# audexdev/Lossless-Audio-Codec

Measured on AMD Instinct MI355X. Metric: encode Msamples/s at 1/2/4/8 MI355X; byte-identical .lac vs CPU ref, higher is better.
Workload: dtype int64

## Files before the change

lossless-audio-codec_amd/csrc/analyze_core.h:

```cpp
#pragma once
#include <type_traits>

#include "lacx_types.h"
#include "x87.h"

namespace lacx {

template <int CH_, int T_>
struct Geo {
    static constexpr int CH = CH_;
    static constexpr int T = T_;
    static constexpr int MAXN = CH_ * T_;
    static constexpr int LV = (CH_ == 16) ? 5 : ((CH_ == 8) ? 4 : 3);
    static constexpr int TPG = 64 / CH_;
    static constexpr int NG = MAXN / 64;
    static constexpr int W256 = 256 / CH_;
    static constexpr int W96 = 96 / CH_;
    static constexpr int MAXP = (MAXN >= 8192) ? 8 : ((MAXN >= 4096) ? 7 : ((MAXN >= 2048) ? 6 : ((MAXN >= 1024) ? 5 : ((MAXN >= 512) ? 4 : 3))));
    static constexpr int NSEG = (2 << MAXP) - 2;
    static constexpr int SW = (T_ < 64) ? T_ : 64;
    static constexpr int NW = (T_ + 63) / 64;
    static_assert(32 % CH_ == 0, "chunk must divide the 96/256 windows");
    static_assert(MAXN % 64 == 0, "whole groups");
};
// ... 788 lines not shown
        if (ZR) {
            n1 = n2;
            n2 = n3;
            n3 = peek_u<G>(sh, (uint32_t)(a + i) + 4u, n);
        }
    }
    ChunkCosts out;
    out.rice = rice;
    out.bin = bin;
    out.zr = zr;
    out.hasrun = hasrun;
    return out;
}

template <class G, bool NARROW, bool ZR = true, bool FULL = false, bool STEADY = false>
LACX_HD void phase_b(Thread<G>& th, const Smem<G>& sh, uint32_t k0) {
    const ChunkCosts cc = phase_b_span<G, NARROW, ZR, FULL ? G::CH : 0, STEADY>(sh, th.n, th.tid, 0, th.cnt, k0);
    th.crice = cc.rice;
    th.cbin = cc.bin;
    th.czr = cc.zr;
    th.chasrun = cc.hasrun;
}

template <class G>
LACX_HD void phase_b_dispatch(Thread<G>& th, const Smem<G>& sh, uint32_t k0, bool narrow, bool zr, bool full, bool steady) {
    auto go = [&](auto narrow_t, auto zr_t) {
        constexpr bool N = decltype(narrow_t)::value, Z = decltype(zr_t)::value;
        if (full) {
            if (steady) phase_b<G, N, Z, true, true>(th, sh, k0); else phase_b<G, N, Z, true, false>(th, sh, k0);
        } else {
            if (steady) phase_b<G, N, Z, false, true>(th, sh, k0); else phase_b<G, N, Z, false, false>(th, sh, k0);
        }
    };
    if (narrow) {
        if (zr) go(std::true_type{}, std::true_type{}); else go(std::true_type{}, std::false_type{});
    } else {
        if (zr) go(std::false_type{}, std::true_type{}); else go(std::false_type{}, std::false_type{});
    }
}
template <class G>
LACX_HD void phase_b_dispatch(Thread<G>& th, const Smem<G>& sh, uint32_t k0, bool narrow, bool zr, bool full) {
    phase_b_dispatch<G>(th, sh, k0, narrow, zr, full, G::T > 64 && th.tid >= 64 && 64 * G::CH >= 256);
}

#ifndef LACX_QUEUED_STEADY
#define LACX_QUEUED_STEADY 1
#endif
template <class G>
LACX_HD void phase_b_queued(Thread<G>& th, const Smem<G>& sh, int t, uint32_t k0, bool narrow, bool zr, bool full) {
    Thread<G> c;
    thread_init(c, th.n, t);
    phase_b_dispatch<G>(c, sh, k0, narrow, zr, full, LACX_QUEUED_STEADY != 0);
    th.crice += c.crice;
    th.cbin += c.cbin;
    th.czr += c.czr;
    th.chasrun |= c.chasrun;
}

LACX_HD uint32_t census_code(uint32_t u);
LACX_HD uint32_t census_shift_sum(uint32_t cen, uint32_t K);

struct RunShape {
    uint32_t nin4, tokens, hasrun, first_in4;
};
template <int CH>
LACX_HD RunShape run_shape(uint32_t E, int32_t f) {
    RunShape r{0u, 0u, 0u, 0u};
#pragma unroll
    for (int i = 0; i < CH; ++i) {
        const uint32_t z = (E >> i) & 1u;
        f = (f + 1) & (int32_t)(0u - z);
        const uint32_t after = E >> (i + 1);
        const uint32_t ahead = (after & 1u) == 0u ? 0u : ((after & 2u) == 0u ? 1u : ((after & 4u) == 0u ? 2u : 3u));
        const uint32_t in4 = z & flag01((uint32_t)f + ahead >= 4u);
        const uint32_t runend = in4 & ((after & 1u) ^ 1u);
        r.nin4 += in4;
        r.tokens += (5u + (((uint32_t)(f - 4)) >> 2)) & (0u - runend);
        r.hasrun |= runend;
        if (i == 0) r.first_in4 = in4;
    }
    return r;
}

template <class G, bool NARROW, bool ZR>
LACX_HD bool phase_b_quick(Thread<G>& th, const Smem<G>& sh) {
    if constexpr (G::T <= 64 || 64 * G::CH <= 256) {
        return false;
    } else {
        const int t = th.tid;
        if (t < 64 || th.cnt != G::CH) return false;
        using Sum = typename std::conditional<NARROW, uint32_t, uint64_t>::type;
        const Sum P0 = (Sum)sh.tabP[t], P1 = (Sum)sh.tabP[t + 1];
        const Sum W0 = (Sum)sh.tabP[t - G::W256], W1 = (Sum)sh.tabP[t - G::W256 + 1];
        const uint32_t c0 = (uint32_t)th.a, c1 = c0 + (uint32_t)G::CH;
        const uint32_t km = kmean_t<NARROW>(P0, c1);
        uint32_t ok = flag01(km == kmean_t<NARROW>(P1, c0));
        const uint32_t Llo = (uint32_t)(((P0 - W1) + 128u) >> 8), Lhi = (uint32_t)(((P1 - W0) + 128u) >> 8);
        const uint32_t Ulo = (3u * Llo + 3u) >> 2, Uhi = (3u * Lhi + 3u) >> 2;
        const uint32_t Dlo = Llo + (Llo + 3u) / 3u + 1u, Dhi = Lhi + (Lhi + 3u) / 3u + 1u;
        const uint64_t Xlo = NARROW ? (uint64_t)((uint32_t)P0 + (c0 >> 1)) : (uint64_t)P0 + (c0 >> 1);
        const uint64_t Xhi = NARROW ? (uint64_t)((uint32_t)P1 + (c1 >> 1)) : (uint64_t)P1 + (c1 >> 1);
        const uint32_t act_never = flag01(Xhi < (uint64_t)c0), act_always = flag01(Xlo >= (uint64_t)c1);
        const uint32_t up_always = flag01(Xhi < (uint64_t)Ulo * c0), up_never = flag01(Xlo >= (uint64_t)Uhi * c1);
        const uint32_t dn_always = flag01(Xlo >= (uint64_t)Dhi * c1), dn_never = flag01(Xhi < (uint64_t)Dlo * c0);
        ok &= act_never | (act_always & (up_always | up_never) & (dn_always | dn_never));
        const int32_t drift = (int32_t)((act_never ^ 1u) & up_always) - (int32_t)((act_never ^ 1u) & dn_always);
        const uint32_t d0 = window_flags<G>(sh.tabF, t), din = sh.tabF[t], dout = sh.tabF[t - G::W96];
        const int32_t l0 = (int32_t)(d0 & 0xFFFFu), z0 = (int32_t)(d0 >> 16);
        const uint32_t big_always = flag01(l0 - (int32_t)(dout & 0xFFFFu) >= 72), big_never = flag01(l0 + (int32_t)(din & 0xFFFFu) < 72);
        uint32_t sml_always, sml_never;
        {
            const uint32_t zin = sh.tabZM[t], zout = sh.tabZM[t - G::W96];
            int32_t z = z0, zmin = z0, zmax = z0;
#pragma unroll
            for (int i = 0; i + 1 < G::CH; ++i) {
                z += (int32_t)((zin >> i) & 1u) - (int32_t)((zout >> i) & 1u);
                zmin = z < zmin ? z : zmin;
                zmax = z > zmax ? z : zmax;
            }
            sml_always = flag01(zmin >= 77);
            sml_never = flag01(zmax < 77);
        }
        ok &= big_always | (big_never & (sml_always | sml_never));
        int32_t bias = drift + (int32_t)big_always - (int32_t)((big_always ^ 1u) & sml_always);
        bias = bias < -1 ? -1 : (bias > 1 ? 1 : bias);
        int bk = (int)km + bias;
        bk = bk < 0 ? 0 : (bk > 31 ? 31 : bk);
        const uint32_t k = (uint32_t)bk;
        uint32_t any = 0;
        Sum ksum = 0;
#pragma unroll
        for (int l = 0; l < G::LV; ++l) {
            any |= th.cs[l];
            ksum += (Sum)(th.cs[l] >> k) << l;
        }
        if (ZR) ok &= flag01((any >> ((k + 3u) < 24u ? (k + 3u) : 24u)) == 0u);
        if (ok == 0u) return false;
        const Sum rice = ksum + (uint32_t)G::CH * (1u + k);
        uint32_t n14 = 0, nbig = (uint32_t)G::CH, small_shifted = 0;
        if (th.umin <= 4u) {
            uint32_t cen = 0;
#pragma unroll
            for (int i = 0; i < G::CH; ++i) cen += census_code(sh.u[i * G::T + t] & 0x3FFFFFFFu);
            n14 = ((cen >> 5) & 31u) + ((cen >> 10) & 31u) + ((cen >> 15) & 31u) + ((cen >> 20) & 31u);
            nbig = (cen >> 25) & 31u;
            small_shifted = census_shift_sum(cen, k);
        }
        th.crice = rice;
        th.cbin = (Sum)(2u * (uint32_t)G::CH + n14 + nbig * (1u + k)) + (ksum - small_shifted);
        RunShape rs{0u, 0u, 0u, 0u};
        if (ZR && th.zmask != 0u)
            rs = run_shape<G::CH>(th.zmask | (((uint32_t)sh.tabUZ[t + 1] & 7u) << G::CH), th.a - 1 - sh.tabNZ[t]);
        const uint32_t nin4 = rs.nin4, tokens = rs.tokens, hasrun = rs.hasrun;
        th.czr = ksum + (Sum)(((uint32_t)G::CH - nin4) * (3u + k) + tokens);
        th.chasrun = hasrun;
        return true;
    }
}

template <class G>
LACX_HD bool phase_b_quick_dispatch(Thread<G>& th, const Smem<G>& sh, bool narrow, bool zr) {
    if (narrow) return zr ? phase_b_quick<G, true, true>(th, sh) : phase_b_quick<G, true, false>(th, sh);
    return zr ? phase_b_quick<G, false, true>(th, sh) : phase_b_quick<G, false, false>(th, sh);
}

LACX_HD uint64_t candidate_lower_bound(uint32_t g_sum, uint32_t aux_sum, uint32_t ends, uint32_t n, int zero_run) {
// ... 611 lines not shown
```

lossless-audio-codec_amd/csrc/device_util.h:

```cpp
#pragma once
#include <hip/hip_runtime.h>

#include "analyze_core.h"
#include "kernels.h"

namespace lacx {

#ifdef LACX_STAMPS
extern __device__ unsigned long long g_stamp_acc[40];
#define STAMP(k)                                                        \
    do {                                                                \
        const unsigned long long _now = __builtin_amdgcn_s_memtime();   \
        stamp_acc[k] += _now - stamp_prev;                              \
        stamp_prev = _now;                                              \
    } while (0)
#define STAMP_PARAMS , unsigned long long* stamp_acc, unsigned long long& stamp_prev
#define STAMP_ARGS , stamp_acc, stamp_prev
#else
#define STAMP(k) do { } while (0)
#define STAMP_PARAMS
#define STAMP_ARGS
#endif
constexpr int kDppRowShr1 = 0x111, kDppRowShr2 = 0x112, kDppRowShr4 = 0x114, kDppRowShr8 = 0x118;
constexpr int kDppRowBcast15 = 0x142, kDppRowBcast31 = 0x143;
// ... 111 lines not shown
    v |= dpp_mov<kDppRowShr2, 0xF>(0u, v);
    v |= dpp_mov<kDppRowShr4, 0xF>(0u, v);
    v |= dpp_mov<kDppRowShr8, 0xF>(0u, v);
    v |= dpp_mov<kDppRowBcast15, 0xA>(0u, v);
    return v;
}
__device__ __forceinline__ uint64_t half_scan_min_u64(uint64_t v) {
    auto step = [](uint64_t a, uint32_t lo, uint32_t hi) {
        const uint64_t b = ((uint64_t)hi << 32) | lo;
        return b < a ? b : a;
    };
#define LACX_MIN_STEP(CTRL, MASK) \
    v = step(v, dpp_mov<CTRL, MASK>(0xFFFFFFFFu, (uint32_t)v), dpp_mov<CTRL, MASK>(0xFFFFFFFFu, (uint32_t)(v >> 32)))
    LACX_MIN_STEP(kDppRowShr1, 0xF);
    LACX_MIN_STEP(kDppRowShr2, 0xF);
    LACX_MIN_STEP(kDppRowShr4, 0xF);
    LACX_MIN_STEP(kDppRowShr8, 0xF);
    LACX_MIN_STEP(kDppRowBcast15, 0xA);
#undef LACX_MIN_STEP
    return v;
}
__device__ __forceinline__ uint64_t half_sum_u64(uint64_t v) { return half_last_u64(half_scan_add_u64(v)); }
__device__ __forceinline__ uint32_t half_sum_u32(uint32_t v) { return half_last_u32(half_scan_add_u32(v)); }
__device__ __forceinline__ uint32_t half_or_u32(uint32_t v) { return half_last_u32(half_scan_or_u32(v)); }
template <int SW> constexpr auto slot_last_u32 = SW == 64 ? &wave_last_u32 : &half_last_u32;
template <int SW> constexpr auto slot_last_u64 = SW == 64 ? &wave_last_u64 : &half_last_u64;
template <int SW> constexpr auto slot_scan_add_u32 = SW == 64 ? &wave_scan_add_u32 : &half_scan_add_u32;
template <int SW> constexpr auto slot_scan_add_u64 = SW == 64 ? &wave_scan_add_u64 : &half_scan_add_u64;
template <int SW> constexpr auto slot_scan_max_i32 = SW == 64 ? &wave_scan_max_i32 : &half_scan_max_i32;
template <int SW> constexpr auto slot_scan_or_u32 = SW == 64 ? &wave_scan_or_u32 : &half_scan_or_u32;
template <int SW> constexpr auto slot_scan_min_u64 = SW == 64 ? &wave_scan_min_u64 : &half_scan_min_u64;
template <int SW> constexpr auto slot_sum_u64 = SW == 64 ? &wave_sum_u64 : &half_sum_u64;
template <int SW> constexpr auto slot_sum_u32 = SW == 64 ? &wave_sum_u32 : &half_sum_u32;
template <int SW> constexpr auto slot_or_u32 = SW == 64 ? &wave_or_u32 : &half_or_u32;
template <int SW>
__device__ __forceinline__ uint32_t slot_first_u32(uint32_t v) {
    static_assert(SW == 64 || SW == 32, "the wave or one of its halves");
    if constexpr (SW == 64) {
        return (uint32_t)__builtin_amdgcn_readfirstlane((int)v);
    } else {
        const uint32_t lo = (uint32_t)__builtin_amdgcn_readlane((int)v, 0), hi = (uint32_t)__builtin_amdgcn_readlane((int)v, 32);
        return upper_half() ? hi : lo;
    }
}
template <int SW>
__device__ __forceinline__ uint64_t slot_ballot(bool pred) {
    const unsigned long long m = __ballot(pred);
    if constexpr (SW == 64) {
        return m;
    } else {
        return upper_half() ? (uint32_t)(m >> 32) : (uint32_t)m;
    }
}
template <int SW>
__device__ __forceinline__ uint32_t slot_rank(uint64_t m) {
    if constexpr (SW == 64) {
        return __builtin_amdgcn_mbcnt_hi((uint32_t)(m >> 32), __builtin_amdgcn_mbcnt_lo((uint32_t)m, 0u));
    } else {
        return (uint32_t)__popc((uint32_t)m & ((1u << (threadIdx.x & 31u)) - 1u));
    }
}

template <int LOG>
__device__ __forceinline__ uint32_t seg_sum_u32(uint32_t v) {
    if (LOG >= 1) v += dpp_mov<kDppRowShr1, 0xF>(0u, v);
    if (LOG >= 2) v += dpp_mov<kDppRowShr2, 0xF>(0u, v);
    if (LOG >= 3) v += dpp_mov<kDppRowShr4, 0xF>(0u, v);
    if (LOG >= 4) v += dpp_mov<kDppRowShr8, 0xF>(0u, v);
    if (LOG >= 5) v += dpp_mov<kDppRowBcast15, 0xA>(0u, v);
    if (LOG >= 6) v += dpp_mov<kDppRowBcast31, 0xC>(0u, v);
    return v;
}
__device__ __forceinline__ uint32_t seg_sum_u32(uint32_t v, int log2_lanes) {
    switch (log2_lanes) {
        case 1: return seg_sum_u32<1>(v);
        case 2: return seg_sum_u32<2>(v);
        case 3: return seg_sum_u32<3>(v);
        case 4: return seg_sum_u32<4>(v);
        case 5: return seg_sum_u32<5>(v);
        default: return seg_sum_u32<6>(v);
    }
}

template <class G>
struct ScanRegs {
    uint64_t v, inc;
    int32_t z, zinc;
};

template <class G, class M>
__device__ __forceinline__ void scan_pz_part1(M& sh, int tid, ScanRegs<G>& r) {
    const int lane = tid & 63, wave = tid >> 6;
    r.v = sh.tabP[tid];
    r.z = sh.tabNZ[tid];
    const uint64_t inc = slot_scan_add_u64<G::SW>(r.v);
    const int32_t zinc = slot_scan_max_i32<G::SW>(r.z);
    r.inc = inc;
    r.zinc = zinc;
    if (lane == G::SW - 1) {
        sh.wtotP[wave] = inc;
        sh.wtotZ[wave] = zinc;
    }
}

template <class G, class M>
__device__ __forceinline__ uint64_t scan_pz_part2(M& sh, int tid, const ScanRegs<G>& r) {
    const int lane = tid & 63, wave = tid >> 6;
    uint64_t base = 0, total = 0;
    int32_t zbase = -1;
#pragma unroll
    for (int w = 0; w < G::NW; ++w) {
        const uint64_t pw = sh.wtotP[w];
        const int32_t z = sh.wtotZ[w];
        total += pw;
        if (w < wave) {
            base += pw;
            zbase = z > zbase ? z : zbase;
        }
    }
    int32_t zprev = __shfl_up(r.zinc, 1, G::SW);
    if (lane == 0) zprev = -1;
    sh.tabP[tid] = base + r.inc - r.v;
    sh.tabNZ[tid] = zprev > zbase ? zprev : zbase;
    if (tid == G::T - 1) {
        sh.tabP[G::T] = base + r.inc;
        sh.tabNZ[G::T] = r.zinc > zbase ? r.zinc : zbase;
    }
    return total;
}

template <class G>
__device__ __forceinline__ void plane_totals_wave(const Thread<G>& th, uint32_t* planeTot, uint32_t* planeTot256,
                                                  int tid, int first_plane = 0) {
    const int lane = tid & 63, wave = tid >> 6;
    uint32_t any = 0;
#pragma unroll
    for (int l = 0; l < G::LV; ++l) any |= th.cs[l];
    if constexpr (G::SW == 32) {
        const int nplanes = 32 - __clz((int)slot_or_u32<32>(any));
        uint32_t mine = 0;
        for (int b = 0; b < nplanes; ++b) {
            uint32_t tot = 0;
#pragma unroll
            for (int l = 0; l < G::LV; ++l) tot += (uint32_t)__popc((uint32_t)slot_ballot<32>((th.cs[l] >> b) & 1u)) << l;
            if (lane == b) mine = tot;
        }
        static_assert(G::SW != 32 || G::W256 == G::SW, "the slot is its own first 256 samples");
        if (lane < nplanes) {
            if (lane >= first_plane) atomicAdd(&planeTot[lane], mine);
            atomicAdd(&planeTot256[lane], mine);
        }
        return;
    }
    const int nplanes = 32 - __clz((int)wave_or_u32(any));
    const uint64_t m256 = (G::W256 >= 64) ? ~0ull : ((1ull << (G::W256 & 63)) - 1ull);
    uint32_t mine = 0, mine256 = 0;
    const bool first256 = wave == 0;
    for (int b = first256 ? 0 : first_plane; b < nplanes; ++b) {
        uint32_t tot = 0, tot256 = 0;
#pragma unroll
        for (int l = 0; l < G::LV; ++l) {
            const uint64_t m = __ballot((th.cs[l] >> b) & 1u);
            tot += (uint32_t)__popcll(m) << l;
            if (first256) tot256 += (uint32_t)__popcll(m & m256) << l;
        }
        if (lane == b) {
// ... 176 lines not shown
```

lossless-audio-codec_amd/csrc/k_analyze.hip:

```cpp
#include <hip/hip_runtime.h>

#include <cstdlib>
#include <mutex>

#include "emit_device.h"
#include "kernels_internal.h"

namespace lacx {

#ifdef LACX_STAMPS
__device__ unsigned long long g_stamp_acc[40];
#endif

#ifdef LACX_TEST_HOOKS
#define LACX_HOOK(prm, bits) (((prm).debug_skip & (bits)) != 0u)
#else
#define LACX_HOOK(prm, bits) false
#endif

struct PendingSlot {
    long long idx;
    uint32_t done, silent;
};

// ... 46 lines not shown
            }
            asm volatile("s_waitcnt vmcnt(0)" ::: "memory");
            __syncthreads();
            if (tid == 0) __hip_atomic_store(&t->state, tmpl_key, __ATOMIC_RELEASE, __HIP_MEMORY_SCOPE_AGENT);
        }
    }
    if (defer) {
        if (tid == 0) {
            defer->idx = idx;
            defer->done = done ? 1u : 0u;
            defer->silent = LACX_HOOK(prm, 8192u) ? 1u : 0u;
        }
        return;
    }
    asm volatile("s_waitcnt vmcnt(0)" ::: "memory");
    __syncthreads();
    if (tid == 0) {
        if (done) fa.emitted[idx] = 2u;
        if (!LACX_HOOK(prm, 8192u)) rec_store(&fa.ready_rec[idx], done ? 1ull : 2ull);
    }
}

__device__ __forceinline__ void publish_pending(const FuseArgs& fa, PendingSlot& pend, int tid) {
    if (tid == 0) {
        const long long idx = pend.idx;
        if (idx >= 0) {
            if (pend.done) fa.emitted[idx] = 2u;
            if (!pend.silent) rec_store(&fa.ready_rec[idx], pend.done ? 1ull : 2ull);
        }
        pend.idx = -1;
    }
}

template <class G>
__device__ __forceinline__ void score_candidate_wave(Smem<G>& sh, int cand, uint32_t n, int zero_run, uint32_t k0,
                                                     const uint32_t* planeTot, const unsigned long long* acc, int lane,
                                                     bool ksums, uint32_t kmask) {
    uint64_t key = ~0ull;
    if (ksums) {
        if (lane < 16 && ((kmask >> lane) & 1u)) key = (((uint64_t)planeTot[lane] + (uint64_t)n * (uint64_t)(1 + lane)) << 4) | (uint64_t)lane;
    } else {
        const int b = 29 - lane;
        const uint64_t w = (lane < 30) ? ((uint64_t)planeTot[b] << b) : 0ull;
        const uint64_t tk = slot_scan_add_u64<G::SW>(w);
        if (lane >= 14 && lane < 30 && ((kmask >> b) & 1u)) key = (((tk >> b) + (uint64_t)n * (uint64_t)(1 + b)) << 4) | (uint64_t)b;
    }
    const uint64_t best_key = slot_last_u64<G::SW>(slot_scan_min_u64<G::SW>(key));
    if (lane == 0) {
        const uint64_t sbits = best_key >> 4;
        const uint32_t sk = (uint32_t)(best_key & 15u);
        const uint64_t rice = acc[0], bin = acc[1];
        const uint32_t hasrun = acc[3] != 0;
        const uint64_t zr = (zero_run && hasrun) ? acc[2] : rice;
        const uint64_t a = rice < sbits ? rice : sbits;
        const uint64_t c = zr < bin ? zr : bin;
        const uint64_t best = a < c ? a : c;
        if (sh.best_cand < 0 || best < sh.best_bits || (best == sh.best_bits && cand < sh.best_cand)) {
            sh.best_cand = cand;
            sh.best_bits = best;
            sh.best_rice = rice;
            sh.best_zr = zr;
            sh.best_bin = bin;
            sh.best_static = sbits;
            sh.best_k0 = k0;
            sh.best_sk = sk;
            sh.best_hasrun = hasrun;
        }
    }
}

template <int SW>
__device__ __forceinline__ uint32_t initial_k_wave(const uint32_t* planes256, uint32_t n, int lane, bool ksums) {
    const uint32_t m = n < 256u ? n : 256u;
    uint64_t key = ~0ull;
    if (ksums) {
        if (lane <= 12) key = (((uint64_t)planes256[lane] + (uint64_t)m * (uint64_t)(1 + lane)) << 4) | (uint64_t)lane;
    } else {
        const int b = 29 - lane;
        const uint64_t w = (lane < 30) ? ((uint64_t)planes256[b] << b) : 0ull;
        const uint64_t tk = slot_scan_add_u64<SW>(w);
        if (lane >= 17 && lane < 30) key = (((tk >> b) + (uint64_t)m * (uint64_t)(1 + b)) << 4) | (uint64_t)b;
    }
    return (uint32_t)(slot_last_u64<SW>(slot_scan_min_u64<SW>(key)) & 15u);
}

template <class G>
__device__ __forceinline__ void slot_sync() {
    if constexpr (G::T <= 64) {
        asm volatile("s_waitcnt lgkmcnt(0)" ::: "memory");
    } else {
        __syncthreads();
    }
}

template <class G>
__device__ __forceinline__ void analyze_slot(unsigned char* smem_raw, const AnalyzeParams& prm, uint32_t n_in,
                                             const SlotSrc& src, int64_t start, const LpcSet* __restrict__ lpc_slot,
                                             ChannelPlan* __restrict__ plan_out, int tid, const FuseArgs& fuse,
                                             const long long fuse_idx, const bool fuse_flag_byte,
                                             const uint32_t fuse_flag_value, PendingSlot* pend) {
    Smem<G>& sh = *reinterpret_cast<Smem<G>*>(smem_raw);
    const uint32_t n = n_in;
#ifdef LACX_STAMPS
    unsigned long long stamp_acc[40];
    for (int k = 0; k < 40; ++k) stamp_acc[k] = 0;
    unsigned long long stamp_prev = __builtin_amdgcn_s_memtime();
    const unsigned long long stamp_rt0 = __builtin_amdgcn_s_memrealtime();
#endif
    Thread<G> th;
    thread_init(th, n, tid);
    const uint32_t chunk_bits = stage_samples(th, sh, src, start);
    {
        const bool wave_silent = slot_ballot<G::SW>(chunk_bits != 0u) == 0ull;
        if ((tid & 63) == 0) sh.wtotF[tid >> 6] = wave_silent ? 0u : 1u;
    }
    for (int i = tid; i < (int)(sizeof(LpcSet) / 2); i += G::T)
        reinterpret_cast<uint16_t*>(&sh.lpc)[i] = reinterpret_cast<const uint16_t*>(lpc_slot)[i];
    if (tid < 32) {
        sh.planeTot[0][tid] = sh.planeTot[1][tid] = 0;
        sh.planeTot256[0][tid] = sh.planeTot256[1][tid] = 0;
    }
    if (tid < 4) sh.acc[0][tid] = sh.acc[1][tid] = 0;
    if constexpr (G::T >= 33) {
        if (tid < 33) (&sh.lbacc[0][0])[tid] = 0;
    } else {
        for (int i = tid; i < 33; i += G::T) (&sh.lbacc[0][0])[i] = 0;
    }
    if (tid < 2) sh.has4[tid] = 0;
    if (tid == 0) {
        sh.best_cand = -1;
        sh.tabUZ[G::T] = sh.tabUZ[G::T + 1] = 0;
    }
    if (pend) asm volatile("s_waitcnt vmcnt(0)" ::: "memory");
    slot_sync<G>();
    if (pend) publish_pending(fuse, *pend, tid);
    STAMP(0);

    auto run_pass1 = [&](const bool real) {
        asm volatile("" : "+v"(th.a));
        const bool lpc_off = LACX_HOOK(prm, 16u);
        const uint32_t per_thread = 34u * (uint32_t)G::CH;
        const int32_t left = (int32_t)n - (int32_t)((tid >> 6) * 64 * G::CH);
        const uint32_t valid = left <= 0 ? 0u : (left >= G::SW * G::CH ? (uint32_t)(G::SW * G::CH) : (uint32_t)left);
        const uint32_t beyond = (uint32_t)(G::SW * G::CH) - valid;
        auto reduce_pair = [&](int c0, const BoundPartials& b0, bool two, const BoundPartials& b1) {
            const uint32_t lo = per_thread - b0.msum, hi = two ? per_thread - b1.msum : 0u;
            const uint32_t g2 = slot_sum_u32<G::SW>(lo | (hi << 16));
            const uint32_t cnt0 = slot_sum_u32<G::SW>(bound_counts<G::CH>(b0));
            const uint32_t cnt1 = two ? slot_sum_u32<G::SW>(bound_counts<G::CH>(b1)) : 0u;
            if ((tid & 63) == 0 && real) {
#pragma unroll
                for (int h = 0; h < 2; ++h) {
                    if (h == 0 || two) {
                        const uint32_t g = h ? (g2 >> 16) : (g2 & 0xFFFFu);
                        const uint32_t cnt = h ? cnt1 : cnt0;
                        const uint32_t nz = cnt & 0x7FFu, n4 = (cnt >> 11) & 0x7FFu, ends = cnt >> 22;
                        atomicAdd(&sh.lbacc[c0 + h][0], g - nz - beyond);
                        atomicAdd(&sh.lbacc[c0 + h][1], (nz - beyond) + (n4 << 16));
                        atomicAdd(&sh.lbacc[c0 + h][2], ends);
                    }
                }
            }
        };
        {
            BoundPartials bf[6];
            if (n == (uint32_t)G::MAXN) pass1_bounds_fixed<G, true>(th, sh, bf);
// ... 117 lines not shown
                sh.bqcount = 0;
                int next = best_key == ~0ull ? -1 : (int)(best_key & 15u);
                if (next >= 0 && !LACX_HOOK(prm, 128u) && candidate_pruned(best_key >> 4, next, sh.best_bits, sh.best_cand)) next = -1;
                sh.next_cand = next;
            }
        }
        STAMP(1);
        slot_sync<G>();
        STAMP(4);
        const int cand = sh.next_cand;
        if (cand < 0) break;
        tried |= 1u << cand;
        asm volatile("" : "+v"(th.a));
        uint32_t* pt = sh.planeTot[parity];
        uint32_t* pt256 = sh.planeTot256[parity];
        unsigned long long* acc = sh.acc[parity];
        {
            uint32_t ures[G::CH];
            phase_r_residual(th, sh, cand, ures);
            phase_r_store(th, sh, ures);
        }
        ScanRegs<G> sr;
        scan_pz_part1(sh, tid, sr);
        STAMP(3);
        slot_sync<G>();
        const uint64_t total_u = scan_pz_part2(sh, tid, sr);
        const bool narrow = total_u < kNarrowLimit;
        const bool ksums = narrow && !LACX_HOOK(prm, 262144u);
        const uint32_t kmask = !LACX_HOOK(prm, 1048576u) ? static_k_candidates<G::SW>(total_u, n, tid & 63) : 0xFFFFu;
        if (!LACX_HOOK(prm, 1u)) {
            if (ksums) ksums_wave(th, pt, pt256, tid, kmask);
            else plane_totals_wave(th, pt, pt256, tid, kmask ? (int)__builtin_ctz(kmask) : 0);
        }
        if (tid < 64) {
            const uint32_t k0w = initial_k_wave<G::SW>(pt256, n, tid, ksums);
            if (tid == 0) sh.cur_k0 = k0w;
        }
        STAMP(6);
        if (LACX_HOOK(prm, 2u)) {
            sh.tabF[tid] = 0;
            th.has4 = 1u;
        } else if (narrow) {
            phase_a<G, true>(th, sh);
        } else {
            phase_a<G, false>(th, sh);
        }
        if (slot_ballot<G::SW>(th.has4 != 0u) != 0ull && (tid & 63) == 0) sh.has4[parity] = 1u;
        STAMP(8);
        slot_sync<G>();
        STAMP(10);
        const uint32_t k0 = sh.cur_k0;
        asm volatile("" : "+v"(th.tid));
        if (LACX_HOOK(prm, 4u)) {
            th.crice = th.cbin = th.czr = 1;
            th.chasrun = 0;
        } else {
            const bool zr = prm.zero_run && sh.has4[parity] != 0u;
            const bool full = n == (uint32_t)G::MAXN;
            if (G::T <= 64 || LACX_HOOK(prm, 524288u)) {
                phase_b_dispatch<G>(th, sh, k0, narrow, zr, full);
                if ((uint32_t)th.a >= n) {
                    th.crice = th.cbin = th.czr = 0;
                    th.chasrun = 0;
                }
            } else {
                const bool live = (uint32_t)th.a < n;
                bool quick = false;
                if (tid >= 64 && live) quick = phase_b_quick_dispatch<G>(th, sh, narrow, zr);
                if (!quick) {
                    th.crice = th.cbin = th.czr = 0;
                    th.chasrun = 0;
                }
                if (tid >= 64) {
                    const unsigned long long slow = __ballot(live && !quick);
                    if (slow != 0ull) {
                        uint32_t base = 0;
                        if ((tid & 63) == 0) base = atomicAdd(&sh.bqcount, (uint32_t)__popcll(slow));
                        base = (uint32_t)__builtin_amdgcn_readfirstlane((int)base);
                        if (live && !quick) sh.bqueue[base + __builtin_amdgcn_mbcnt_hi((uint32_t)(slow >> 32), __builtin_amdgcn_mbcnt_lo((uint32_t)slow, 0u))] = (uint16_t)tid;
                    }
                }
                STAMP(11);
                slot_sync<G>();
                if (tid < 64) {
                    if (live) phase_b_dispatch<G>(th, sh, k0, narrow, zr, full, false);
                } else {
                    const int w = tid >> 6;
                    const int order = (w & 3) ? (w - 1 - (w >> 2)) : (11 + (w >> 2));
                    const uint32_t qn = sh.bqcount;
                    for (uint32_t e0 = (uint32_t)order * 64u; e0 < qn; e0 += 15u * 64u) {
                        const uint32_t e = e0 + (uint32_t)(tid & 63);
                        if (e < qn) phase_b_queued<G>(th, sh, (int)sh.bqueue[e], k0, narrow, zr, full);
                    }
                }
            }
        }
        STAMP(12);
        {
            const uint64_t r0 = slot_sum_u64<G::SW>(th.crice);
            const uint64_t r1 = slot_sum_u64<G::SW>(th.cbin);
            const uint64_t r2 = slot_sum_u64<G::SW>(th.czr);
            const uint32_t r3 = slot_or_u32<G::SW>(th.chasrun);
            if ((tid & 63) == 0) {
                atomicAdd(&acc[0], (unsigned long long)r0);
                atomicAdd(&acc[1], (unsigned long long)r1);
                atomicAdd(&acc[2], (unsigned long long)r2);
                atomicAdd(&acc[3], (unsigned long long)r3);
            }
        }
        STAMP(13);
        slot_sync<G>();
        STAMP(14);
        pending = cand;
        pending_k0 = k0;
        pending_ksums = ksums;
        pending_kmask = kmask;
        parity ^= 1;
    }

    STAMP(15);
    asm volatile("" : "+v"(tid), "+v"(th.tid), "+v"(th.a));
    const int best = sh.best_cand;
    int max_p = 0;
    if (prm.partitioning && n >= (uint32_t)kMinPartition) max_p = max_partition_order(n);
    const int nseg = max_p > 0 ? ((2 << max_p) - 2) : 0;
    PartMem<G>& pm = sh.xp.part;
    auto clear_partition_scratch = [&]() {
        for (int i = tid; i < nseg; i += G::T) {
            pm.segacc[i][0] = pm.segacc[i][1] = pm.segacc[i][2] = 0;
            pm.segrun[i] = 0;
        }
        if (tid <= G::MAXP) pm.pbits[tid] = 0;
    };
    if (best == pending && !LACX_HOOK(prm, 16384u)) {
        clear_partition_scratch();
        slot_sync<G>();
    } else {
        phase_r(th, sh, best);
        ScanRegs<G> sr;
        scan_pz_part1(sh, tid, sr);
        slot_sync<G>();
        clear_partition_scratch();
        scan_pz_part2(sh, tid, sr);
        slot_sync<G>();
    }
    const bool pnarrow = sh.tabP[G::T] < kNarrowLimit;
    STAMP(16);
    if (max_p > 0) {
        {
            constexpr int kLog = G::TPG == 4 ? 2 : (G::TPG == 8 ? 3 : 4);
            static_assert(G::TPG == 4 || G::TPG == 8 || G::TPG == 16, "lanes per 64-sample group");
            uint32_t words[15];
            packed_planes(th, words);
            const bool last = (tid & (G::TPG - 1)) == G::TPG - 1;
#pragma unroll
            for (int w = 0; w < 15; ++w) {
                const uint32_t v = seg_sum_u32<kLog>(words[w]);
                if (last) pm.grp[w][tid / G::TPG] = v;
            }
            if (tid < 15) pm.grp[tid][G::NG] = 0;
        }
        slot_sync<G>();
        {
            constexpr int NW = G::NW;
            const int wave = tid >> 6, lane = tid & 63;
            for (int w = wave; w < 15; w += NW) wave_exclusive_scan_u32<G::SW>(pm.grp[w], G::NG + 1, lane);
        }
// ... 475 lines not shown
```

Baseline: 24950.

## Split phase-B slow-path chunks across four-lane quads for CH16 narrow slots

For 16-sample chunks in the narrow path, the queued slow-path chunk cost evaluation (plus the first 64 chunks) is redistributed so that each chunk is handled by a quad of four lanes, each lane taking four samples. Prefix sums within a quad come from DPP quad broadcasts, and per-sample zero-run state is recomputed from bitmasks rather than carried serially. The goal is to cut per-lane serial work and the load imbalance of one lane walking sixteen samples. In exchange, each lane does redundant window-mask and shared-memory loads, and the code has more instructions.

```diff
diff --git a/lossless-audio-codec_amd/csrc/analyze_core.h b/lossless-audio-codec_amd/csrc/analyze_core.h
--- a/lossless-audio-codec_amd/csrc/analyze_core.h
+++ b/lossless-audio-codec_amd/csrc/analyze_core.h
@@ -894,6 +894,140 @@
     return r;
 }
 
+LACX_HD int32_t zeros_ending_at(uint32_t E, int i, int32_t f0) {
+    const uint32_t nz = ~E & ((2u << i) - 1u);
+    return nz == 0u ? f0 + i + 1 : i - (31 - clz32(nz));
+}
+LACX_HD uint32_t zeros_ahead(uint32_t E, int i) {
+    const uint32_t after = E >> (i + 1);
+    return (after & 1u) == 0u ? 0u : ((after & 2u) == 0u ? 1u : ((after & 4u) == 0u ? 2u : 3u));
+}
+
+template <class G>
+struct WindowMasks {
+    uint32_t has96, in[G::W96];
+};
+template <class G, bool STEADY = false>
+LACX_HD WindowMasks<G> window_masks(int t) {
+    WindowMasks<G> m;
+    m.has96 = STEADY ? 0xFFFFFFFFu : 0u - flag01(t >= G::W96);
+#pragma unroll
+    for (int k = 1; k <= G::W96; ++k) m.in[k - 1] = STEADY ? 0xFFFFFFFFu : 0u - flag01(t >= k);
+    return m;
+}
+template <class G>
+LACX_HD uint32_t flags_before(const Smem<G>& sh, int t, int i, const WindowMasks<G>& m, uint32_t* fin, uint32_t* fout) {
+    const uint32_t below = ((1u << i) - 1u) * 0x00010001u;
+    const int t96 = (t - G::W96) & (int)m.has96;
+    uint32_t f[G::W96];
+#pragma unroll
+    for (int k = 1; k <= G::W96; ++k) f[k - 1] = sh.tabF[(t - k) & (int)m.in[k - 1]];
+    const uint32_t lin = sh.tabLM[t], zin = sh.tabZM[t], lout = sh.tabLM[t96], zout = sh.tabZM[t96];
+    *fin = lin | (zin << 16);
+    *fout = (lout | (zout << 16)) & m.has96;
+    uint32_t D = 0;
+#pragma unroll
+    for (int k = 0; k < G::W96; ++k) D += f[k] & m.in[k];
+    const uint32_t in = *fin & below, out = *fout & below;
+    D += (uint32_t)__builtin_popcount(in & 0xFFFFu) + ((uint32_t)__builtin_popcount(in >> 16) << 16);
+    D -= (uint32_t)__builtin_popcount(out & 0xFFFFu) + ((uint32_t)__builtin_popcount(out >> 16) << 16);
+    return D;
+}
+
+struct SampleCosts {
+    uint32_t rice, bin, zr, runend;
+};
+
+template <bool ZR = true, bool STEADY = false>
+LACX_HD SampleCosts phase_b_sample(uint32_t P, uint32_t W, uint32_t D, uint32_t c, uint32_t u, uint32_t E, int i, int32_t f0,
+                                   uint32_t k0) {
+    const uint32_t cc = c ? c : 1u;
+    const uint32_t kb = biased_k<true, STEADY>(kmean32(P, cc), P, W, D, cc);
+    const uint32_t kin = (STEADY || c != 0u) ? kb : k0;
+    SampleCosts out;
+    const uint32_t rc = (u >> kin) + 1u + kin;
+    out.rice = rc;
+    out.bin = 2u + ((u <= 4u) ? (u < 1u ? u : 1u) : rc);
+    out.zr = 0;
+    out.runend = 0;
+    if (ZR) {
+        const uint32_t z = (E >> i) & 1u;
+        const int32_t f = zeros_ending_at(E, i, f0);
+        const uint32_t ahead = zeros_ahead(E, i);
+        const uint32_t in4 = z & flag01((uint32_t)f + ahead >= 4u);
+        const uint32_t esc = 1u << ((kin + 3u) < 24u ? (kin + 3u) : 24u);
+        const uint32_t plain = 2u + ((u > esc) ? 32u : rc);
+        const uint32_t token = 5u + (((uint32_t)(f - 4)) >> 2);
+        const uint32_t runend = in4 & (((E >> (i + 1)) & 1u) ^ 1u);
+        out.zr = (plain & (in4 - 1u)) | (token & (0u - runend));
+        out.runend = runend;
+    }
+    return out;
+}
+
+template <int SPAN>
+struct LaneIn {
+    uint32_t u[SPAN], tap[SPAN];
+    uint32_t usum, tapsum;
+    uint32_t P0, W0;
+    uint32_t D, fin, fout, E;
+    int32_t f0;
+};
+template <class G, int SPAN, bool STEADY = false>
+LACX_HD LaneIn<SPAN> phase_b_lane_in(const Smem<G>& sh, uint32_t n, int t, int i0) {
+    LaneIn<SPAN> in;
+    uint32_t live[SPAN];
+#pragma unroll
+    for (int k = 0; k < SPAN; ++k) live[k] = 0u - flag01((uint32_t)(t * G::CH + i0 + k) < n);
+    const uint32_t has256 = STEADY ? 0xFFFFFFFFu : 0u - flag01(t >= G::W256);
+    const WindowMasks<G> wm = window_masks<G, STEADY>(t);
+    const int t256 = (t - G::W256) & (int)has256;
+#pragma unroll
+    for (int k = 0; k < SPAN; ++k) {
+        in.u[k] = sh.u[(i0 + k) * G::T + t];
+        in.tap[k] = sh.u[(i0 + k) * G::T + t256];
+    }
+    const uint32_t P0 = (uint32_t)sh.tabP[t], W0 = (uint32_t)sh.tabP[t256];
+    const uint32_t z0 = sh.tabUZ[t], z1 = sh.tabUZ[t + 1];
+    const int32_t nz = sh.tabNZ[t];
+    in.D = flags_before<G>(sh, t, i0, wm, &in.fin, &in.fout);
+    in.usum = in.tapsum = 0;
+#pragma unroll
+    for (int k = 0; k < SPAN; ++k) {
+        in.u[k] &= live[k];
+        in.tap[k] &= live[k] & has256;
+        in.usum += in.u[k];
+        in.tapsum += in.tap[k];
+    }
+    in.P0 = P0;
+    in.W0 = W0 & has256;
+    in.E = z0 | ((z1 & 7u) << G::CH);
+    in.f0 = t * G::CH - 1 - nz;
+    return in;
+}
+
+template <class G, int SPAN, bool ZR, bool STEADY>
+LACX_HD SampleCosts phase_b_lane(const LaneIn<SPAN>& in, uint32_t P, uint32_t W, uint32_t n, int t, int i0, uint32_t k0) {
+    SampleCosts sum{0u, 0u, 0u, 0u};
+    uint32_t D = in.D;
+#pragma unroll
+    for (int k = 0; k < SPAN; ++k) {
+        const int i = i0 + k;
+        const uint32_t c = (uint32_t)(t * G::CH + i);
+        const SampleCosts sc = phase_b_sample<ZR, STEADY>(P, W, D, c, in.u[k], in.E, i, in.f0, k0);
+        const uint32_t add = 0u - flag01(c < n);
+        sum.rice += sc.rice & add;
+        sum.bin += sc.bin & add;
+        sum.zr += sc.zr & add;
+        sum.runend |= sc.runend & add;
+        P += in.u[k];
+        W += in.tap[k];
+        D += (in.fin >> i) & 0x00010001u;
+        D -= (in.fout >> i) & 0x00010001u;
+    }
+    return sum;
+}
+
 template <class G, bool NARROW, bool ZR>
 LACX_HD bool phase_b_quick(Thread<G>& th, const Smem<G>& sh) {
     if constexpr (G::T <= 64 || 64 * G::CH <= 256) {
diff --git a/lossless-audio-codec_amd/csrc/device_util.h b/lossless-audio-codec_amd/csrc/device_util.h
--- a/lossless-audio-codec_amd/csrc/device_util.h
+++ b/lossless-audio-codec_amd/csrc/device_util.h
@@ -217,6 +217,11 @@
     }
 }
 
+__device__ __forceinline__ uint32_t quad_exclusive_scan_u32(uint32_t v, uint32_t place ) {
+    const uint32_t v0 = dpp_mov<0x00, 0xF>(0u, v), v1 = dpp_mov<0x55, 0xF>(0u, v), v2 = dpp_mov<0xAA, 0xF>(0u, v);
+    return (place > 0u ? v0 : 0u) + (place > 1u ? v1 : 0u) + (place > 2u ? v2 : 0u);
+}
+
 template <class G>
 struct ScanRegs {
     uint64_t v, inc;
diff --git a/lossless-audio-codec_amd/csrc/k_analyze.hip b/lossless-audio-codec_amd/csrc/k_analyze.hip
--- a/lossless-audio-codec_amd/csrc/k_analyze.hip
+++ b/lossless-audio-codec_amd/csrc/k_analyze.hip
@@ -152,6 +152,44 @@
         if (lane >= 17 && lane < 30) key = (((tk >> b) + (uint64_t)m * (uint64_t)(1 + b)) << 4) | (uint64_t)b;
     }
     return (uint32_t)(slot_last_u64<SW>(slot_scan_min_u64<SW>(key)) & 15u);
+}
+
+template <class G, bool ZR>
+__device__ __forceinline__ void phase_b_quads(Thread<G>& th, const Smem<G>& sh, uint32_t k0, int tid_in) {
+    static_assert(G::CH == 16 && G::NW == 16, "four lanes of four samples per chunk, sixteen waves");
+    const int tid = opaque_i32(tid_in);
+    const uint32_t n = th.n;
+    const uint32_t place = (uint32_t)tid & 3u, quad = ((uint32_t)tid >> 2) & 15u;
+    const int i0 = (int)place * 4;
+    const uint32_t wave = (uint32_t)__builtin_amdgcn_readfirstlane(tid >> 6);
+    const uint32_t total = 64u + sh.bqcount;
+    uint32_t rice = 0, bin = 0, zr = 0, hasrun = 0;
+    auto trip = [&](auto steady_tag, uint32_t e0) {
+        constexpr bool STEADY = decltype(steady_tag)::value;
+        const uint32_t e = e0 + quad;
+        const uint32_t have = 0u - flag01(e < total);
+        const uint32_t queued = STEADY ? sh.bqueue[(e - 64u) & have] : 0u;
+        const int t = STEADY ? (int)((queued & have) | (64u & ~have)) : (int)(e & have);
+        const LaneIn<4> in = phase_b_lane_in<G, 4, STEADY>(sh, n, t, i0);
+        const uint32_t P = in.P0 + quad_exclusive_scan_u32(in.usum, place);
+        const uint32_t W = in.W0 + quad_exclusive_scan_u32(in.tapsum, place);
+        const SampleCosts sc = phase_b_lane<G, 4, ZR, STEADY>(in, P, W, n, t, i0, k0);
+        rice += sc.rice & have;
+        bin += sc.bin & have;
+        if (ZR) {
+            zr += sc.zr & have;
+            hasrun |= sc.runend & have;
+        }
+    };
+    uint32_t group = wave;
+    for (uint32_t round = 0; group * 16u < total; ++round) {
+        if (group < 4u) trip(std::false_type{}, group * 16u); else trip(std::true_type{}, group * 16u);
+        group = (round & 1u) ? (round + 1u) * 16u + wave : (round + 1u) * 16u + 15u - wave;
+    }
+    th.crice += rice;
+    th.cbin += bin;
+    th.czr += zr;
+    th.chasrun |= hasrun;
 }
 
 template <class G>
@@ -435,7 +473,11 @@
                 }
                 STAMP(11);
                 slot_sync<G>();
-                if (tid < 64) {
+                if (G::CH == 16 && narrow && !LACX_HOOK(prm, 256u)) {
+                    if constexpr (G::CH == 16) {
+                        if (zr) phase_b_quads<G, true>(th, sh, k0, tid); else phase_b_quads<G, false>(th, sh, k0, tid);
+                    }
+                } else if (tid < 64) {
                     if (live) phase_b_dispatch<G>(th, sh, k0, narrow, zr, full, false);
                 } else {
                     const int w = tid >> 6;
```

Measured after the change: 25330 (median of 5 runs). 1.5% higher.
